# laclouis5/StructureDetector

Hardware: AMD Instinct MI355X
Metric: images/sec (train fwd+bwd) and decode us/img at 512x512 (higher is better)
Workload: dtype f32

## Files before the change

structuredetector_amd/csrc/sd_conv.hip:

```cpp
#include <string.h>
#include "sd_common.h"
#include "sd_mfma.h"
#include "sd_conv_rows.h"

#ifndef SD_S2_LPT
#define SD_S2_LPT 1
#endif
namespace sd {


#ifndef SD_IGEMM_DMA
#define SD_IGEMM_DMA 1
#endif
#ifndef SD_ABLATE_HOT
#define SD_ABLATE_HOT 0
#endif
#ifndef SD_ABLATE_STORE
#define SD_ABLATE_STORE 0
#endif
#ifndef SD_ABLATE_PATCH
#define SD_ABLATE_PATCH 0
#endif
#if SD_ABLATE_HOT || SD_ABLATE_STORE || SD_ABLATE_PATCH || defined(SD_PP_ABL) || defined(SD_RS_ABL)
#warning "timing-only ablation build: this libsdnet_hip.so computes WRONG RESULTS; the Python loader refuses it unless SDNET_ALLOW_ABLATION=1"
#endif
#ifdef SD_DECODE_TRACE
#define SD_TRACE_FLAG 8
#else
#define SD_TRACE_FLAG 0
#endif
#if defined(SD_PP_TRACE) || defined(SD_SB_TRACE)
#undef SD_TRACE_FLAG
#define SD_TRACE_FLAG 8
#endif
#if defined(SD_PP_ABL) || defined(SD_RS_ABL) || defined(SD_SB_ABL) || defined(SD_SHAPE_EXP) || defined(SD_W16_ABL) || defined(SD_SR_ABL) || defined(SD_SF_ABL)
#define SD_EXPERIMENT_FLAG 16
#else
#define SD_EXPERIMENT_FLAG 0
#endif
void sd_nn_set_pool_pair(int v);
extern "C" int sd_build_flags(void) { return (SD_ABLATE_HOT ? 1 : 0) | (SD_ABLATE_STORE ? 2 : 0) | (SD_ABLATE_PATCH ? 4 : 0) | SD_TRACE_FLAG | SD_EXPERIMENT_FLAG; }

#ifndef SD_SHAPE_EXP
#define SD_SHAPE_EXP 0
#else
#define SD_SHAPE_EXP_BUILD 1
#endif
__device__ __forceinline__ f32x16 mfma_shape_exp(bf16x8 a, bf16x8 b, f32x16 c) {
    f32x4 c0 = __builtin_shufflevector(c, c, 0, 1, 2, 3), c1 = __builtin_shufflevector(c, c, 4, 5, 6, 7);
    c0 = __builtin_amdgcn_mfma_f32_16x16x32_bf16(a, b, c0, 0, 0, 0);
    c1 = __builtin_amdgcn_mfma_f32_16x16x32_bf16(b, a, c1, 0, 0, 0);
    c[0] = c0[0]; c[1] = c0[1]; c[2] = c0[2]; c[3] = c0[3]; c[4] = c1[0]; c[5] = c1[1]; c[6] = c1[2]; c[7] = c1[3];
    return c;
}
#define SD_MFMA_BF16(BIT, a, b, c) (((SD_SHAPE_EXP) & (BIT)) ? mfma_shape_exp(a, b, c) : __builtin_amdgcn_mfma_f32_32x32x16_bf16(a, b, c, 0, 0, 0))

#ifndef SD_IGEMM_LATE_DMA
#define SD_IGEMM_LATE_DMA 0
#endif
constexpr int NBUF = 2;
constexpr int BM = 128, BK = 32, LDK = BK;

struct ConvArgs {
    const void* x;
    const void* w;
    void* y;
    const float* scale;
    const float* shift;
    const void* res;
    int B, Hi, Wi, Ck, Ho, Wo, Nn, R, S;
    int mul, div, off, rsign;
    int relu, res_up2;
    int M, nk, kchunks;
    int splits;
    float* part;
    const float* bn_x;
    const float* bn_y;
    const float *bn_mean, *bn_invstd, *bn_gamma, *bn_beta;
    int bn_relu;
    float* stat;
    int pt_tw_log2, pt_pw, pt_pieces, pt_rolling, pt_flip;
    int pt_strip_log2;
    int par;
    const uint16_t* head_w;
    const float* head_b;
    float* head_y;
    int head_co;
};

__device__ __attribute__((aligned(128))) float g_zero_line[64];


__device__ __forceinline__ void s2_tile(int bid, int nwg, int n_tiles, int off, int& cls, int& tq, int& n_idx, int& tile_m) {
    if (SD_S2_LPT && (nwg & 31) == 0) {
        const int xcd = bid & 7, pos = bid >> 3, per = nwg >> 5;
        const int k4 = pos / per, within = xcd * per + (pos - k4 * per);
        cls = (off & 1) ? (k4 == 0 ? 3 : k4 == 3 ? 0 : k4) : k4;
        tq = within / n_tiles; n_idx = within - tq * n_tiles;
    } else {
        const int tile = xcd_remap(bid, nwg), tm = tile / n_tiles;
        cls = tm & 3; tq = tm >> 2; n_idx = tile - tm * n_tiles;
    }
    tile_m = 4 * tq + cls;
}


__device__ __forceinline__ float f4c(const float4& v, int t) { return t == 0 ? v.x : (t == 1 ? v.y : (t == 2 ? v.z : v.w)); }

struct BnRed4 { float4 mu, is, ga, be, s, q; };
__device__ __forceinline__ void bnred4_init(BnRed4& b, const ConvArgs& p, int n) {
    b.mu = *reinterpret_cast<const float4*>(p.bn_mean + n); b.is = *reinterpret_cast<const float4*>(p.bn_invstd + n);
    b.ga = b.be = b.s = b.q = make_float4(0.f, 0.f, 0.f, 0.f);
    if (p.bn_relu == 2) { b.ga = *reinterpret_cast<const float4*>(p.bn_gamma + n); b.be = *reinterpret_cast<const float4*>(p.bn_beta + n); }
}
__device__ __forceinline__ void bnred4_add(BnRed4& b, const ConvArgs& p, float4 g, int64_t m, int n) {
    const int64_t i = m * p.Nn + n;
    const float4 xv = *reinterpret_cast<const float4*>(p.bn_x + i);
    const float4 xh = make_float4((xv.x - b.mu.x) * b.is.x, (xv.y - b.mu.y) * b.is.y, (xv.z - b.mu.z) * b.is.z, (xv.w - b.mu.w) * b.is.w);
    if (p.bn_relu == 1) {
        const float4 yy = *reinterpret_cast<const float4*>(p.bn_y + i);
        g.x = yy.x > 0.f ? g.x : 0.f; g.y = yy.y > 0.f ? g.y : 0.f; g.z = yy.z > 0.f ? g.z : 0.f; g.w = yy.w > 0.f ? g.w : 0.f;
    } else if (p.bn_relu == 3) {
        const uint8_t mb = reinterpret_cast<const uint8_t*>(p.bn_y)[i >> 2];
        g.x = (mb & 1) ? g.x : 0.f; g.y = (mb & 2) ? g.y : 0.f; g.z = (mb & 4) ? g.z : 0.f; g.w = (mb & 8) ? g.w : 0.f;
    } else if (p.bn_relu == 2) {
        g.x = (xh.x * b.ga.x + b.be.x) > 0.f ? g.x : 0.f; g.y = (xh.y * b.ga.y + b.be.y) > 0.f ? g.y : 0.f;
        g.z = (xh.z * b.ga.z + b.be.z) > 0.f ? g.z : 0.f; g.w = (xh.w * b.ga.w + b.be.w) > 0.f ? g.w : 0.f;
    }
    b.s.x += g.x; b.s.y += g.y; b.s.z += g.z; b.s.w += g.w;
    b.q.x += g.x * xh.x; b.q.y += g.y * xh.y; b.q.z += g.z * xh.z; b.q.w += g.w * xh.w;
}
template <int LPR>
__device__ __forceinline__ void bnred4_wave_sum(BnRed4& b) {
#pragma unroll
    for (int o = LPR; o < 64; o <<= 1) {
        b.s.x += __shfl_xor(b.s.x, o); b.s.y += __shfl_xor(b.s.y, o); b.s.z += __shfl_xor(b.s.z, o); b.s.w += __shfl_xor(b.s.w, o);
        b.q.x += __shfl_xor(b.q.x, o); b.q.y += __shfl_xor(b.q.y, o); b.q.z += __shfl_xor(b.q.z, o); b.q.w += __shfl_xor(b.q.w, o);
    }
}

#define SD_BNRED_TERM(v, m, n, S, Q)                                                               \
    {                                                                                              \
        const float xv_ = p.bn_x[(int64_t)(m) * p.Nn + (n)];                                       \
        const float xh_ = (xv_ - bmu) * bis;                                                       \
        float g_ = (v);                                                                            \
        if (p.bn_relu == 1) g_ = p.bn_y[(int64_t)(m) * p.Nn + (n)] > 0.f ? g_ : 0.f;               \
        else if (p.bn_relu == 3) g_ = ((reinterpret_cast<const uint8_t*>(p.bn_y)[((int64_t)(m) * p.Nn + (n)) >> 2] >> ((n) & 3)) & 1) ? g_ : 0.f; \
        else if (p.bn_relu == 2) g_ = (xh_ * bga + bbe) > 0.f ? g_ : 0.f;                          \
        S += g_; Q += g_ * xh_;                                                                    \
    }

template <int BN, int MODE, bool BF16 = false>
__global__ __launch_bounds__(256, 2) void k_conv_igemm(ConvArgs p) {
    constexpr bool STEM = (MODE == 1);
    using T = typename std::conditional<BF16, uint16_t, float>::type;
    constexpr int KE = BF16 ? 64 : 32;
    constexpr int VE = BF16 ? 8 : 4;
    const T* const px_ = reinterpret_cast<const T*>(p.x);
    const T* const pw_ = reinterpret_cast<const T*>(p.w);
    const T* const zero_ = reinterpret_cast<const T*>(g_zero_line);
    constexpr int NT = BN / 64;
    __shared__ __attribute__((aligned(16))) float As0[BM * LDK];
    __shared__ __attribute__((aligned(16))) float As1[BM * LDK];
    __shared__ __attribute__((aligned(16))) float Bs0[BN * LDK];
    __shared__ __attribute__((aligned(16))) float Bs1[BN * LDK];
    __shared__ int orow[BM];
    __shared__ int rrow[BM];

    const int tid = threadIdx.x, lane = tid & 63, wave = tid >> 6;
    const int n_tiles = p.Nn / BN;
    const int tile = xcd_remap(blockIdx.x, gridDim.x);
// ... 4304 lines not shown
    a.pt_rolling = a.Wo == 128;
    a.pt_pw = a.pt_rolling ? 144 : a.Wo + 2;
    a.pt_pieces = a.pt_rolling ? 36 : cdiv((th + 2) * a.pt_pw, 16);
    a.pt_flip = a.rsign < 0;
    return a.pt_pieces * 256 <= (a.pt_rolling ? PT_FLOATS : PT_STAGE_FLOATS);
}

static thread_local int g_patch_narrow = 2;
static int patch_tile_bn(ConvArgs& a, int BN, int mode, bool bf16) {
    ConvArgs t = a;
    if (conv_patch_geometry(t, BN, mode, bf16, false, g_patch_min_tiles)) { a = t; return BN; }
    if (BN == 128 && (bf16 ? g_patch_narrow >= 2 : g_patch_narrow >= 1)) {
        t = a;
        if (conv_patch_geometry(t, 64, mode, bf16, true, g_patch_min_tiles)) { a = t; return 64; }
    }
    return 0;
}

static thread_local int g_rows64_min_units = 192;
static bool conv_rows64_geometry(const ConvArgs& a, int mode, RowsArgs& r) {
    if (mode != 0 || a.Ck != 64 || a.Nn != 64 || a.R != 3 || a.S != 3 || a.mul != 1 || a.div != 1 || a.splits > 1) return false;
    if (!((a.rsign == 1 && a.off == -1) || (a.rsign == -1 && a.off == 1))) return false;
    if (a.Ho != a.Hi || a.Wo != a.Wi || a.Wo % 128 || a.res_up2 || a.bn_x) return false;
    r = RowsArgs{};
    r.B = a.B; r.H = a.Ho; r.W = a.Wo; r.segs = a.Wo / 128;
    const int cols = r.B * r.segs;
    r.rows = std::min(r.H, std::max(8, cdiv(r.H * cols, 256)));
    r.units_per_col = cdiv(r.H, r.rows);
    r.nunits = cols * r.units_per_col;
    if (r.nunits < g_rows64_min_units || (g_rows64_min_units > 1 && r.rows < 16)) return false;
    r.x = (const uint16_t*)a.x; r.w = (const uint16_t*)a.w; r.y = (uint16_t*)a.y; r.scale = a.scale; r.shift = a.shift;
    r.res = (const uint16_t*)a.res; r.stat = a.stat; r.relu = a.relu; r.flip = a.rsign < 0;
    return true;
}

static thread_local int g_rows16 = 1;
static bool conv_rows16_args(const RowsArgs& r) { return g_rows16 && !r.stat; }

static thread_local int g_rowsf32_min_units = 192;
static thread_local int g_stem_fwd_blocks = 512;
static bool conv_rowsf32_geometry(const ConvArgs& a, int mode, RowsArgsF& r) {
    if (mode != 0 || a.Ck != 64 || a.Nn != 64 || a.R != 3 || a.S != 3 || a.mul != 1 || a.div != 1 || a.splits > 1) return false;
    if (!((a.rsign == 1 && a.off == -1) || (a.rsign == -1 && a.off == 1))) return false;
    if (a.Ho != a.Hi || a.Wo != a.Wi || a.Wo % 64 || a.res_up2 || a.bn_x) return false;
    r = RowsArgsF{};
    r.B = a.B; r.H = a.Ho; r.W = a.Wo; r.segs = a.Wo / 64;
    const int cols = r.B * r.segs;
    r.rows = std::min(r.H, std::max(8, cdiv(r.H * cols, 256)));
    r.units_per_col = cdiv(r.H, r.rows);
    r.nunits = cols * r.units_per_col;
    if (r.nunits < g_rowsf32_min_units || (g_rowsf32_min_units > 1 && r.rows < 16)) return false;
    r.x = (const float*)a.x; r.w = (const float*)a.w; r.y = (float*)a.y; r.scale = a.scale; r.shift = a.shift;
    r.res = (const float*)a.res; r.stat = a.stat; r.relu = a.relu; r.flip = a.rsign < 0;
    return true;
}

static thread_local int g_pp_min_tiles = 200;
static thread_local int g_pp_strips = 1;
static bool conv_pp_geometry(ConvArgs& a, int mode, int min_tiles) {
    if (a.Nn % 128 || a.M % PP_BM || (a.M / PP_BM) * (a.Nn / 128) < min_tiles || a.res_up2) return false;
    a.pt_strip_log2 = 0;
    int l2 = 0;
    while ((1 << l2) < a.Wo) ++l2;
    if (g_pp_strips && (1 << l2) == a.Wo && a.Wo >= 128 && a.Wo <= 4096 && a.Ho % 4 == 0) {
        if (!SD_CONV_PATCH || mode != 0 || a.R != 3 || a.S != 3 || a.mul != 1 || a.div != 1 || a.splits > 1) return false;
        if (!((a.rsign == 1 && a.off == -1) || (a.rsign == -1 && a.off == 1))) return false;
        if (a.Ho != a.Hi || a.Wo != a.Wi || a.Ck % 32) return false;
        a.pt_tw_log2 = 6; a.pt_strip_log2 = l2 - 6; a.pt_rolling = 0; a.pt_pw = 66; a.pt_pieces = cdiv(6 * 66, 16); a.pt_flip = a.rsign < 0;
        return true;
    }
    return conv_patch_geometry(a, 128, mode, true, false, 1) && !a.pt_rolling;
}

static thread_local int g_stem_fwd_ring = 1;
static thread_local int g_igemm_big_bf16 = 0;
static int igemm_big_tiles(const ConvArgs& a, int BN, int mode) {
    if (!SD_IGEMM_BIG || (BN != 128 && !SD_IGEMM_BIG64 && !(SD_IGEMM_BIG64_S2 && mode == 2)) || (mode != 0 && mode != 2) || a.splits > 1) return 0;
    if (a.R * a.S * a.Ck < 512) return 0;
    const int m_per = mode == 2 ? a.M / 4 : a.M;
    const int big_tiles = (mode == 2 ? 4 : 1) * cdiv(m_per, BMB) * (a.Nn / BN);
    return (big_tiles >= 512 && (mode != 2 || m_per % BMB == 0)) ? big_tiles : 0;
}

enum ConvFamily {
    CONV_STREAM1X1,
    CONV_ROWS16,
    CONV_ROWS_BF16,
    CONV_ROWS_F32,
    CONV_PP,
    CONV_PP_HEAD,
    CONV_PATCH,
    CONV_PATCH_ROLL,
    CONV_IGEMM_BIG,
    CONV_IGEMM,
};

struct ConvPlan {
    ConvFamily family;
    bool bf16;
    int BN, mode;
    int grid_x, grid_y, block;
    size_t lds;
    int stat_rows;
    ConvArgs a;
    RowsArgs ra;
    RowsArgsF rf;
};

static ConvPlan plan_conv(const ConvArgs& a, bool bf16, bool stem = false) {
    ConvPlan p{};
    p.bf16 = bf16;
    p.a = a;
    p.BN = (a.Nn % 128 == 0) ? 128 : 64;
    p.mode = stem ? 1 : (a.par ? 2 : (a.div > 1 ? 3 : 0));
    p.grid_y = 1; p.block = 256;
    if (!stem && bf16) {
        if (conv1x1_stream_geometry(a, p.mode) && conv1x1_stream_args(a)) {
            p.family = CONV_STREAM1X1;
            p.grid_x = std::min(512, cdiv(a.M / (a.Ck == 64 ? 32 : 16), 4));
            return p;
        }
        if (conv_rows64_geometry(a, p.mode, p.ra)) {
            p.family = conv_rows16_args(p.ra) ? CONV_ROWS16 : CONV_ROWS_BF16;
            p.grid_x = std::min(p.ra.nunits, 256); p.lds = RS_LDS_BYTES; p.stat_rows = p.ra.nunits;
            return p;
        }
        ConvArgs t = a;
        if (conv_pp_geometry(t, p.mode, g_pp_min_tiles)) {
            p.a = t;
            p.family = a.head_y ? CONV_PP_HEAD : CONV_PP;
            p.BN = 128; p.grid_x = (a.M / PP_BM) * (a.Nn / 128); p.block = 512; p.lds = PP_LDS_FLOATS * sizeof(float); p.stat_rows = a.M / PP_BM;
            return p;
        }
    }
    if (!stem && !bf16 && conv_rowsf32_geometry(a, p.mode, p.rf)) {
        p.family = CONV_ROWS_F32;
        p.grid_x = std::min(p.rf.nunits, 256); p.lds = RF_LDS_BYTES; p.stat_rows = p.rf.nunits;
        return p;
    }
    if (!stem) {
        if (const int PBN = patch_tile_bn(p.a, p.BN, p.mode, bf16)) {
            p.family = p.a.pt_rolling ? CONV_PATCH_ROLL : CONV_PATCH;
            p.BN = PBN; p.grid_x = (a.M / BMB) * (a.Nn / PBN); p.stat_rows = cdiv(a.M, BMB);
            return p;
        }
    }
    if (const int big_tiles = (!bf16 || (g_igemm_big_bf16 && p.BN == 128)) ? igemm_big_tiles(a, p.BN, p.mode) : 0) {
        p.family = CONV_IGEMM_BIG;
        p.grid_x = big_tiles; p.stat_rows = cdiv(a.M, BMB);
        return p;
    }
    p.family = CONV_IGEMM;
    p.grid_x = cdiv(a.M, BM) * (a.Nn / p.BN); p.grid_y = a.splits > 1 ? a.splits : 1; p.stat_rows = a.splits > 1 ? 0 : cdiv(a.M, BM);
    return p;
}

static const char* conv_plan_name(const ConvPlan& p, char* buf, size_t n) {
    const char* tf = p.bf16 ? "true" : "false";
    switch (p.family) {
    case CONV_STREAM1X1: return p.a.Ck == 64 ? "k_conv1x1_stream_bf16<64, 2>" : "k_conv1x1_stream_bf16<128, 1>";
    case CONV_ROWS16: return "k_conv3x3_c64_rows16_bf16";
    case CONV_ROWS_BF16: return "k_conv3x3_c64_rows_bf16";
    case CONV_ROWS_F32: return "k_conv3x3_c64_rows_f32";
    case CONV_PP: return "k_conv3x3_bf16_pp";
    case CONV_PP_HEAD: return "k_conv3x3_bf16_pp_head";
    case CONV_PATCH: snprintf(buf, n, "k_conv3x3_patch<%d, %s>", p.BN, tf); return buf;
    case CONV_PATCH_ROLL: snprintf(buf, n, "k_conv3x3_patch_roll<%d, %s>", p.BN, tf); return buf;
    case CONV_IGEMM_BIG: snprintf(buf, n, "k_conv_igemm_big<%d, %d, %s>", p.BN, p.mode, tf); return buf;
    case CONV_IGEMM: snprintf(buf, n, "k_conv_igemm<%d, %d, %s>", p.BN, p.mode, tf); return buf;
    }
    return "";
}

template <auto KERNEL>
static int raise_dynamic_lds(size_t bytes) {
    static thread_local bool raised = false;
    if (!raised) {
        SD_HIP(hipFuncSetAttribute(reinterpret_cast<const void*>(KERNEL), hipFuncAttributeMaxDynamicSharedMemorySize, (int)bytes));
        raised = true;
    }
    return 0;
}

template <int BN, int MODE, bool BF16 = false>
static void launch_tiles(const ConvPlan& p, hipStream_t st) {
    if constexpr ((BN == 128 || (!BF16 && (SD_IGEMM_BIG64 || (SD_IGEMM_BIG64_S2 && MODE == 2)))) && (MODE == 0 || MODE == 2)) {
        if (p.family == CONV_IGEMM_BIG) {
            hipLaunchKernelGGL((k_conv_igemm_big<BN, MODE, BF16>), dim3(p.grid_x), dim3(256), 0, st, p.a);
            return;
        }
    }
    hipLaunchKernelGGL((k_conv_igemm<BN, MODE, BF16>), dim3(p.grid_x, p.grid_y), dim3(256), 0, st, p.a);
}
template <int BN, bool BF16>
static void launch_tiles_mode(const ConvPlan& p, hipStream_t st) {
    if (p.mode == 0) launch_tiles<BN, 0, BF16>(p, st);
    else if (p.mode == 2) launch_tiles<BN, 2, BF16>(p, st);
    else launch_tiles<BN, 3, BF16>(p, st);
}
template <bool BF16>
static void launch_patch(const ConvPlan& p, hipStream_t st) {
    if (p.family == CONV_PATCH_ROLL) {
        if (p.BN == 128) hipLaunchKernelGGL((k_conv3x3_patch_roll<128, BF16>), dim3(p.grid_x), dim3(256), 0, st, p.a);
        else hipLaunchKernelGGL((k_conv3x3_patch_roll<64, BF16>), dim3(p.grid_x), dim3(256), 0, st, p.a);
    } else if (p.BN == 128) hipLaunchKernelGGL((k_conv3x3_patch<128, BF16>), dim3(p.grid_x), dim3(256), 0, st, p.a);
    else hipLaunchKernelGGL((k_conv3x3_patch<64, BF16>), dim3(p.grid_x), dim3(256), 0, st, p.a);
}

static int launch_plan(const ConvPlan& p, hipStream_t st) {
    const ConvArgs& a = p.a;
    SD_REQUIRE(!a.head_y || p.family == CONV_PP_HEAD, SD_ERR_INVALID,
               "sd_conv2d_fwd_bf16_head: this geometry does not take the two-group kernel (ask sd_conv2d_fwd_bf16_head_supported)");
    const dim3 grid(p.grid_x, p.grid_y), block(p.block);
    switch (p.family) {
    case CONV_STREAM1X1:
        if (a.Ck == 64) hipLaunchKernelGGL((k_conv1x1_stream_bf16<64, 2>), grid, block, 0, st, a, a.M / 32);
        else hipLaunchKernelGGL((k_conv1x1_stream_bf16<128, 1>), grid, block, 0, st, a, a.M / 16);
        break;
    case CONV_ROWS16:
    case CONV_ROWS_BF16:
        if (int e = raise_dynamic_lds<k_conv3x3_c64_rows_bf16>(p.lds)) return e;
        if (p.family == CONV_ROWS16) {
            if (int e = launch_rows16_bf16(p.ra, st)) return e;
        } else hipLaunchKernelGGL(k_conv3x3_c64_rows_bf16, grid, block, p.lds, st, p.ra);
        break;
    case CONV_ROWS_F32:
        if (int e = raise_dynamic_lds<k_conv3x3_c64_rows_f32>(p.lds)) return e;
        hipLaunchKernelGGL(k_conv3x3_c64_rows_f32, grid, block, p.lds, st, p.rf);
        break;
    case CONV_PP:
        if (int e = raise_dynamic_lds<k_conv3x3_bf16_pp>(p.lds)) return e;
        hipLaunchKernelGGL(k_conv3x3_bf16_pp, grid, block, p.lds, st, a);
        break;
    case CONV_PP_HEAD:
        if (int e = raise_dynamic_lds<k_conv3x3_bf16_pp_head>(p.lds)) return e;
        hipLaunchKernelGGL(k_conv3x3_bf16_pp_head, grid, block, p.lds, st, a);
        break;
    case CONV_PATCH:
    case CONV_PATCH_ROLL:
        if (p.bf16) launch_patch<true>(p, st); else launch_patch<false>(p, st);
        break;
    case CONV_IGEMM_BIG:
    case CONV_IGEMM:
        if (p.bf16) {
            if (p.BN == 128) launch_tiles_mode<128, true>(p, st); else launch_tiles_mode<64, true>(p, st);
        } else if (p.mode == 1) launch_tiles<64, 1>(p, st);
        else if (p.BN == 128) launch_tiles_mode<128, false>(p, st);
        else launch_tiles_mode<64, false>(p, st);
        break;
    }
    SD_LAUNCH_CHECK();
    if (p.family == CONV_IGEMM && a.splits > 1) {
        if (p.bf16) hipLaunchKernelGGL(k_splitk_reduce<true>, dim3(cdiv((int64_t)a.M * a.Nn / 4, 256)), dim3(256), 0, st, a);
        else hipLaunchKernelGGL(k_splitk_reduce<false>, dim3(cdiv((int64_t)a.M * a.Nn / 4, 256)), dim3(256), 0, st, a);
        SD_LAUNCH_CHECK();
    }
    return 0;
}

static int launch_igemm(const ConvArgs& a, bool stem, hipStream_t st, bool bf16 = false) { return launch_plan(plan_conv(a, bf16, stem), st); }

static thread_local int g_fwd_split_k = 1;
static int fwd_splits(const sd_conv_desc* d, int ke) {
    if (!g_fwd_split_k) return 1;
    const int M = d->B * d->Ho * d->Wo;
    const int BN = (d->Cout % 128 == 0) ? 128 : 64;
    const int tiles = cdiv(M, BM) * (d->Cout / BN);
    const int nk = d->R * d->S * (d->Cin / ke);
    if (tiles >= 256 || nk < 8) return 1;
    int s = std::min(cdiv(512, tiles), nk / 4);
    return std::max(1, std::min(s, 64));
}

static ConvArgs conv_args(const sd_conv_desc* d, int pass, bool bf16) {
    ConvArgs a{};
    const int ke = bf16 ? 64 : BK;
    a.B = d->B; a.R = d->R; a.S = d->S;
    if (pass == 0) {
        a.Hi = d->Hi; a.Wi = d->Wi; a.Ck = d->Cin; a.Ho = d->Ho; a.Wo = d->Wo; a.Nn = d->Cout;
        a.mul = d->stride; a.div = 1; a.off = -d->pad; a.rsign = 1;
        a.splits = fwd_splits(d, ke);
    } else {
        a.Hi = d->Ho; a.Wi = d->Wo; a.Ck = d->Cout; a.Ho = d->Hi; a.Wo = d->Wi; a.Nn = d->Cin;
        a.mul = 1; a.div = d->stride; a.off = d->pad; a.rsign = -1;
    }
    a.M = a.B * a.Ho * a.Wo; a.kchunks = a.Ck / ke; a.nk = a.R * a.S * a.kchunks;
    if (pass == 1) a.par = (d->stride == 2 && d->Hi % 2 == 0 && d->Wi % 2 == 0 && (a.M / 4) % BM == 0) ? 1 : 0;
    return a;
}

static float g_query_operand;
static ConvPlan plan_query(const sd_conv_desc* d, int pass, bool bf16, bool stats) {
    ConvArgs a = conv_args(d, pass, bf16);
    if (stats) { a.stat = &g_query_operand; if (pass == 1) a.bn_x = &g_query_operand; }
    return plan_conv(a, bf16);
}

static int check_conv(const char* what, const sd_conv_desc* d) {
    SD_REQUIRE(d != nullptr, SD_ERR_INVALID, "%s: null descriptor", what);
    SD_REQUIRE(d->B > 0 && d->Hi > 0 && d->Wi > 0 && d->Cin > 0 && d->Cout > 0 && d->R > 0 && d->S > 0 && d->stride > 0 && d->pad >= 0,
// ... 720 lines not shown
    SD_REQUIRE(stem_is_7x7s2(d), SD_ERR_INVALID, "sd_conv2d_stem_wgrad_bf16: the stem is 7x7 / stride 2 / pad 3, 3 -> 64");
    SD_REQUIRE(aligned16(dy_bf16) && aligned16(x_nchw) && d->Wi % 4 == 0, SD_ERR_INVALID,
               "sd_conv2d_stem_wgrad_bf16: dy and the image must be 16-byte aligned and the image width a multiple of 4 (LDS-DMA in 16-byte groups)");
    SD_REQUIRE(workspace_bytes >= sd_conv2d_stem_wgrad_workspace_bytes(d), SD_ERR_WORKSPACE, "sd_conv2d_stem_wgrad_bf16: workspace too small");
    StemArgs a{};
    a.x = x_nchw; a.dy16 = (const uint16_t*)dy_bf16; a.y = (float*)workspace;
    stem_args(a, d);
    a.rg = 64;
    while (a.rg > 8 && d->B * a.tiles_x * cdiv(d->Ho, a.rg) < 512) a.rg >>= 1;
    const int units = d->B * a.tiles_x * cdiv(d->Ho, a.rg);
    const int blocks = std::max(1, std::min(std::min(256, stem_blocks(d)), units));
    hipStream_t st = (hipStream_t)stream;
    static const hipError_t attr_once = hipFuncSetAttribute(reinterpret_cast<const void*>(&k_stem_wgrad_bf16_ring), hipFuncAttributeMaxDynamicSharedMemorySize, (int)SR_LDS_BYTES);
    (void)attr_once;
    hipLaunchKernelGGL(k_stem_wgrad_bf16_ring, dim3(blocks), dim3(256), SR_LDS_BYTES, st, a);
    SD_LAUNCH_CHECK();
    const int64_t n4 = 64 * STEM_K / 4;
    hipLaunchKernelGGL(k_wgrad_reduce_par, dim3(cdiv(n4, 32)), dim3(256), 0, st, (const float*)workspace, dw, n4, blocks, accumulate);
    SD_LAUNCH_CHECK();
    return 0;
}

size_t sd_conv2d_dgrad_bn_reduce_workspace_bytes(const sd_conv_desc* d) {
    if (!d || d->Cin % 64 || d->Cout % 32) return 0;
    const int rows = plan_query(d, 1, false, true).stat_rows;
    return (size_t)(rows + sd_bn_finalize_scratch_rows(rows)) * 2 * d->Cin * sizeof(float);
}

static int conv_dgrad_bn_reduce_any(const char* what, const float* dy, const float* w_t, float* dx, const sd_conv_desc* d, const float* residual,
                                    const float* bn_x, const float* bn_y, int relu, const float* mean, const float* invstd, const float* gamma,
                                    const float* beta, float* dgamma, float* dbeta, int accumulate, float* means_out, double* sums, void* workspace,
                                    size_t workspace_bytes, sd_stream_t stream) {
    if (int e = check_conv(what, d)) return e;
    SD_REQUIRE(dy && w_t && dx && bn_x && mean && invstd && gamma && dgamma && dbeta && (means_out || sums) && workspace, SD_ERR_INVALID,
               "%s: null pointer", what);
    SD_REQUIRE(relu >= 0 && relu <= 3 && ((relu != 1 && relu != 3) || bn_y) && (relu != 2 || beta), SD_ERR_INVALID,
               "%s: relu must be 0, 1 / 3 (need bn_y) or 2 (needs beta)", what);
    SD_REQUIRE(d->Cout % 32 == 0 && d->Cin % 64 == 0, SD_ERR_INVALID, "%s: needs Cout %% 32 == 0 and Cin %% 64 == 0", what);
    SD_REQUIRE(aligned16(dy) && aligned16(w_t) && aligned16(dx) && aligned16(residual) && aligned16(bn_x) && aligned16(bn_y) && aligned16(mean) &&
               aligned16(invstd) && aligned16(gamma) && aligned16(beta) && aligned8(sums), SD_ERR_ALIGN, "%s: pointers must be 16-byte aligned", what);
    SD_REQUIRE(workspace_bytes >= sd_conv2d_dgrad_bn_reduce_workspace_bytes(d), SD_ERR_WORKSPACE, "%s: workspace too small", what);
    ConvArgs a = conv_args(d, 1, false);
    a.x = dy; a.w = w_t; a.y = dx; a.res = residual;
    a.bn_x = bn_x; a.bn_y = bn_y; a.bn_relu = relu; a.bn_mean = mean; a.bn_invstd = invstd; a.bn_gamma = gamma; a.bn_beta = beta;
    a.stat = (float*)workspace;
    const ConvPlan p = plan_conv(a, false);
    if (int e = launch_plan(p, (hipStream_t)stream)) return e;
    const int rows = p.stat_rows;
    if (sums) return sd_bn_bwd_sums((const float*)workspace, rows, (int64_t)a.M, d->Cin, dgamma, dbeta, accumulate, sums,
                                    (float*)workspace + (size_t)rows * 2 * d->Cin, stream);
    return sd_bn_bwd_finalize((const float*)workspace, rows, (int64_t)a.M, d->Cin, dgamma, dbeta, accumulate, means_out,
                              (float*)workspace + (size_t)rows * 2 * d->Cin, stream);
}

int sd_conv2d_dgrad_bn_reduce(const float* dy, const float* w_t, float* dx, const sd_conv_desc* d, const float* residual, const float* bn_x,
                              const float* bn_y, int relu, const float* mean, const float* invstd, const float* gamma, const float* beta,
                              float* dgamma, float* dbeta, int accumulate, float* means_out, void* workspace, size_t workspace_bytes,
                              sd_stream_t stream) {
    SD_REQUIRE(means_out, SD_ERR_INVALID, "sd_conv2d_dgrad_bn_reduce: null pointer");
    return conv_dgrad_bn_reduce_any("sd_conv2d_dgrad_bn_reduce", dy, w_t, dx, d, residual, bn_x, bn_y, relu, mean, invstd, gamma, beta, dgamma, dbeta,
                                    accumulate, means_out, nullptr, workspace, workspace_bytes, stream);
}

int sd_conv2d_dgrad_bn_reduce_sums(const float* dy, const float* w_t, float* dx, const sd_conv_desc* d, const float* residual, const float* bn_x,
                                   const float* bn_y, int relu, const float* mean, const float* invstd, const float* gamma, const float* beta,
                                   float* dgamma, float* dbeta, int accumulate, double* sums, void* workspace, size_t workspace_bytes,
                                   sd_stream_t stream) {
    SD_REQUIRE(sums, SD_ERR_INVALID, "sd_conv2d_dgrad_bn_reduce_sums: null pointer");
    return conv_dgrad_bn_reduce_any("sd_conv2d_dgrad_bn_reduce_sums", dy, w_t, dx, d, residual, bn_x, bn_y, relu, mean, invstd, gamma, beta, dgamma,
                                    dbeta, accumulate, nullptr, sums, workspace, workspace_bytes, stream);
}

#ifdef SD_PP_TRACE
int sd_debug_pp_trace(unsigned long long* out32) { return (int)hipMemcpyFromSymbol(out32, HIP_SYMBOL(sd::g_pp_trace), sizeof(unsigned long long) * 64); }
int sd_debug_stem_trace(unsigned long long* out64) { return (int)hipMemcpyFromSymbol(out64, HIP_SYMBOL(sd::g_stem_trace), sizeof(unsigned long long) * 64); }
int sd_debug_pp_timeline(unsigned long long* out, int blocks) { return (int)hipMemcpyFromSymbol(out, HIP_SYMBOL(sd::g_pp_tl), sizeof(unsigned long long) * 4 * (blocks < 4096 ? blocks : 4096)); }
#endif

int sd_set_option(const char* name, int value) {
    if (name && !strcmp(name, "conv_patch_min_tiles")) { g_patch_min_tiles = value; return 0; }
    if (name && !strcmp(name, "conv_patch_bn64")) { g_patch_bn64 = value; return 0; }
    if (name && !strcmp(name, "conv_pp_min_tiles")) { g_pp_min_tiles = value; return 0; }
    if (name && !strcmp(name, "conv1x1_stream_min_pixels")) { g_conv1x1_stream_min_px = value; return 0; }
    if (name && !strcmp(name, "igemm_big_bf16")) { g_igemm_big_bf16 = value; return 0; }
    if (name && !strcmp(name, "stem_fwd_ring")) { g_stem_fwd_ring = value; return 0; }
    if (name && !strcmp(name, "pool_fwd_pair")) { sd_nn_set_pool_pair(value); return 0; }
    if (name && !strcmp(name, "wgrad_bf16_ring")) { g_wgrad_bf16_ring = value; return 0; }
    if (name && !strcmp(name, "wgrad_f32_ring")) { g_wgrad_f32_ring = value; return 0; }
    if (name && !strcmp(name, "conv_pp_strips")) { g_pp_strips = value; return 0; }
    if (name && !strcmp(name, "conv_patch_narrow")) { g_patch_narrow = value; return 0; }
    if (name && !strcmp(name, "conv_fwd_split_k")) { g_fwd_split_k = value; return 0; }
    if (name && !strcmp(name, "conv_rows64_min_units")) { g_rows64_min_units = value; return 0; }
    if (name && !strcmp(name, "conv_rows16")) { g_rows16 = value; return 0; }
    if (name && !strcmp(name, "conv_rows_f32_min_units")) { g_rowsf32_min_units = value; return 0; }
    if (name && !strcmp(name, "stem_fwd_blocks")) { g_stem_fwd_blocks = value; return 0; }
    sd::set_error("sd_set_option: unknown option '%s'", name ? name : "(null)");
    return SD_ERR_INVALID;
}

const char* sd_conv2d_kernel_name(const sd_conv_desc* d, int pass) {
    static thread_local char name[64];
    if (!d || d->Cin <= 0 || d->Cout <= 0) return "";
    if (pass == 2) {
        const WgradPlan p = plan_wgrad(d, false);
        switch (p.family) {
        case WGRAD_TAPS_RING2: return "k_wgrad3x3_ring2";
        case WGRAD_TAPS_RING: return "k_wgrad3x3_ring";
        case WGRAD_TAPS: return p.roww == 32 ? "k_wgrad3x3<32>" : "k_wgrad3x3<16>";
        default: snprintf(name, sizeof(name), "k_conv_wgrad<%d, %d>", p.TN, p.TC); return name;
        }
    }
    return conv_plan_name(plan_query(d, pass & 15, (pass & 16) != 0, false), name, sizeof(name));
}

}
```

Measured before the change: 872.0.

## Add persistent streaming f32 MFMA kernel for large 1x1 convolutions

Adds a new persistent kernel for f32 1x1 convolutions (stride 1 or 2) and routes large non-bf16 cases to it ahead of the rows/patch/igemm paths. It uses a 4-stage LDS DMA ring with swizzled layout, f32 MFMA, residual prefetch two chunks before the epilogue, and a fused epilogue for BN statistics, scale/shift, residual and relu. The goal is to overlap global loads with compute and amortise launch and tile setup across tiles, in place of the generic implicit-GEMM path. It adds inline-asm wait-count bookkeeping, which risks subtle hazards, and moves ConvArgs into a shared header.

Measured after the change: 874.6, median of 6. No clear change (+0.3%).

```diff
diff --git a/structuredetector_amd/csrc/sd_conv.hip b/structuredetector_amd/csrc/sd_conv.hip
--- a/structuredetector_amd/csrc/sd_conv.hip
+++ b/structuredetector_amd/csrc/sd_conv.hip
@@ -2,6 +2,7 @@
 #include "sd_common.h"
 #include "sd_mfma.h"
 #include "sd_conv_rows.h"
+#include "sd_conv_args.h"
 
 #ifndef SD_S2_LPT
 #define SD_S2_LPT 1
@@ -61,32 +62,6 @@
 constexpr int NBUF = 2;
 constexpr int BM = 128, BK = 32, LDK = BK;
 
-struct ConvArgs {
-    const void* x;
-    const void* w;
-    void* y;
-    const float* scale;
-    const float* shift;
-    const void* res;
-    int B, Hi, Wi, Ck, Ho, Wo, Nn, R, S;
-    int mul, div, off, rsign;
-    int relu, res_up2;
-    int M, nk, kchunks;
-    int splits;
-    float* part;
-    const float* bn_x;
-    const float* bn_y;
-    const float *bn_mean, *bn_invstd, *bn_gamma, *bn_beta;
-    int bn_relu;
-    float* stat;
-    int pt_tw_log2, pt_pw, pt_pieces, pt_rolling, pt_flip;
-    int pt_strip_log2;
-    int par;
-    const uint16_t* head_w;
-    const float* head_b;
-    float* head_y;
-    int head_co;
-};
 
 __device__ __attribute__((aligned(128))) float g_zero_line[64];
 
@@ -4557,8 +4532,20 @@
     return (big_tiles >= 512 && (mode != 2 || m_per % BMB == 0)) ? big_tiles : 0;
 }
 
+static thread_local int g_conv1x1_f32_stream_min_px = 16384;
+static thread_local int g_conv1x1_f32_stream_wide_min_tiles = 256;
+static thread_local int g_conv1x1_f32_stream_blocks = 0;
+static int conv1x1_stream_f32_bn(const ConvArgs& a, int mode) {
+    if (mode != 0 || a.R != 1 || a.S != 1 || a.div != 1 || a.off != 0 || (a.mul != 1 && a.mul != 2) || a.head_y) return 0;
+    if (a.Ck % 64 || a.Nn % 64 || (a.Ck == 512 && a.Nn == 512) || a.M < g_conv1x1_f32_stream_min_px) return 0;
+    if (a.bn_x || a.res_up2 > 1 || (a.res_up2 == 1 && (a.Ho % 2 || a.Wo % 2))) return 0;
+    if (a.stat && (a.splits > 1 || igemm_big_tiles(a, a.Nn % 128 == 0 ? 128 : 64, mode))) return 0;
+    return (a.Nn % 128 == 0 && cdiv(a.M, 128) * (a.Nn / 128) >= g_conv1x1_f32_stream_wide_min_tiles) ? 128 : 64;
+}
+
 enum ConvFamily {
     CONV_STREAM1X1,
+    CONV_STREAM1X1_F32,
     CONV_ROWS16,
     CONV_ROWS_BF16,
     CONV_ROWS_F32,
@@ -4608,6 +4595,13 @@
             return p;
         }
     }
+    if (!stem && !bf16) {
+        if (const int SBN = conv1x1_stream_f32_bn(a, p.mode)) {
+            p.family = CONV_STREAM1X1_F32;
+            p.BN = SBN; p.a.splits = 1; p.grid_x = 0; p.stat_rows = cdiv(a.M, BM);
+            return p;
+        }
+    }
     if (!stem && !bf16 && conv_rowsf32_geometry(a, p.mode, p.rf)) {
         p.family = CONV_ROWS_F32;
         p.grid_x = std::min(p.rf.nunits, 256); p.lds = RF_LDS_BYTES; p.stat_rows = p.rf.nunits;
@@ -4634,6 +4628,7 @@
     const char* tf = p.bf16 ? "true" : "false";
     switch (p.family) {
     case CONV_STREAM1X1: return p.a.Ck == 64 ? "k_conv1x1_stream_bf16<64, 2>" : "k_conv1x1_stream_bf16<128, 1>";
+    case CONV_STREAM1X1_F32: return p.BN == 128 ? "k_conv1x1_stream_f32<128>" : "k_conv1x1_stream_f32<64>";
     case CONV_ROWS16: return "k_conv3x3_c64_rows16_bf16";
     case CONV_ROWS_BF16: return "k_conv3x3_c64_rows_bf16";
     case CONV_ROWS_F32: return "k_conv3x3_c64_rows_f32";
@@ -4691,6 +4686,9 @@
     case CONV_STREAM1X1:
         if (a.Ck == 64) hipLaunchKernelGGL((k_conv1x1_stream_bf16<64, 2>), grid, block, 0, st, a, a.M / 32);
         else hipLaunchKernelGGL((k_conv1x1_stream_bf16<128, 1>), grid, block, 0, st, a, a.M / 16);
+        break;
+    case CONV_STREAM1X1_F32:
+        if (int e = launch_conv1x1_stream_f32(a, p.BN, g_conv1x1_f32_stream_blocks, st)) return e;
         break;
     case CONV_ROWS16:
     case CONV_ROWS_BF16:
@@ -5577,6 +5575,9 @@
     if (name && !strcmp(name, "conv_patch_bn64")) { g_patch_bn64 = value; return 0; }
     if (name && !strcmp(name, "conv_pp_min_tiles")) { g_pp_min_tiles = value; return 0; }
     if (name && !strcmp(name, "conv1x1_stream_min_pixels")) { g_conv1x1_stream_min_px = value; return 0; }
+    if (name && !strcmp(name, "conv1x1_f32_stream_min_pixels")) { g_conv1x1_f32_stream_min_px = value; return 0; }
+    if (name && !strcmp(name, "conv1x1_f32_stream_wide_min_tiles")) { g_conv1x1_f32_stream_wide_min_tiles = value; return 0; }
+    if (name && !strcmp(name, "conv1x1_f32_stream_blocks")) { g_conv1x1_f32_stream_blocks = value; return 0; }
     if (name && !strcmp(name, "igemm_big_bf16")) { g_igemm_big_bf16 = value; return 0; }
     if (name && !strcmp(name, "stem_fwd_ring")) { g_stem_fwd_ring = value; return 0; }
     if (name && !strcmp(name, "pool_fwd_pair")) { sd_nn_set_pool_pair(value); return 0; }
diff --git a/structuredetector_amd/csrc/sd_conv1x1_f32.hip b/structuredetector_amd/csrc/sd_conv1x1_f32.hip
--- /dev/null
+++ b/structuredetector_amd/csrc/sd_conv1x1_f32.hip
@@ -0,0 +1,319 @@
+#include <algorithm>
+#include "sd_common.h"
+#include "sd_mfma.h"
+#include "sd_conv_args.h"
+
+namespace sd {
+
+constexpr int S1_BM = 128, S1_BK = 16, S1_NST = 4, S1_PAW = 2;
+
+static __device__ __attribute__((aligned(128))) float g_s1_zero_line[64];
+
+constexpr int s1_vmcnt_imm(int n) { return (n & 15) | (7 << 4) | (15 << 8) | ((n >> 4) << 14); }
+
+__device__ __forceinline__ f32x4 s1_load16_async(const float* src) {
+    f32x4 v = {0.f, 0.f, 0.f, 0.f};
+#if defined(__HIP_DEVICE_COMPILE__)
+    asm volatile("global_load_dwordx4 %0, %1, off" : "=&v"(v) : "v"(src) : "memory");
+#else
+    (void)src;
+#endif
+    return v;
+}
+template <int N>
+__device__ __forceinline__ void s1_wait_loads(f32x4 (&r)[16]) {
+#if defined(__HIP_DEVICE_COMPILE__)
+    asm volatile("s_waitcnt %16"
+                 : "+v"(r[0]), "+v"(r[1]), "+v"(r[2]), "+v"(r[3]), "+v"(r[4]), "+v"(r[5]), "+v"(r[6]), "+v"(r[7]), "+v"(r[8]), "+v"(r[9]),
+                   "+v"(r[10]), "+v"(r[11]), "+v"(r[12]), "+v"(r[13]), "+v"(r[14]), "+v"(r[15])
+                 : "n"(s1_vmcnt_imm(N))
+                 : "memory");
+#endif
+}
+template <int N>
+__device__ __forceinline__ void s1_wait_loads(f32x4 (&r)[8]) {
+#if defined(__HIP_DEVICE_COMPILE__)
+    asm volatile("s_waitcnt %8"
+                 : "+v"(r[0]), "+v"(r[1]), "+v"(r[2]), "+v"(r[3]), "+v"(r[4]), "+v"(r[5]), "+v"(r[6]), "+v"(r[7])
+                 : "n"(s1_vmcnt_imm(N))
+                 : "memory");
+#endif
+}
+__device__ __forceinline__ void s1_lds_barrier() {
+#if defined(__HIP_DEVICE_COMPILE__)
+    asm volatile("s_waitcnt lgkmcnt(0)\n\ts_barrier" ::: "memory");
+#endif
+}
+
+template <int OFF>
+__device__ __forceinline__ void s1_lds_write32(uint32_t addr, float v) {
+#if defined(__HIP_DEVICE_COMPILE__)
+    asm volatile("ds_write_b32 %0, %1 offset:%2" :: "v"(addr), "v"(v), "n"(OFF) : "memory");
+#else
+    (void)addr; (void)v;
+#endif
+}
+__device__ __forceinline__ float s1_lds_read32(uint32_t addr) {
+    float v = 0.f;
+#if defined(__HIP_DEVICE_COMPILE__)
+    asm volatile("ds_read_b32 %0, %1\n\ts_waitcnt lgkmcnt(0)" : "=v"(v) : "v"(addr) : "memory");
+#else
+    (void)addr;
+#endif
+    return v;
+}
+
+template <int BN, bool FULL, int NS>
+__device__ __forceinline__ void s1_epilogue(const ConvArgs& p, f32x16 (&acc)[2][BN / 64], f32x4 (&R)[NS], uint32_t T, uint32_t statred,
+                                            int m0, int n0, int tile_m, const f32x4 sc4, const f32x4 sh4, int wave, int lane) {
+    constexpr int WC = BN / 2, NTW = WC / 32, LPR = WC / 4, RPI = 64 / LPR, IPP = 8 / RPI;
+    const int fr = lane & 31, fh = lane >> 5;
+    const int wm0 = (wave >> 1) * 64, wn0 = (wave & 1) * WC;
+    if (p.stat) {
+        float sv[NTW], qv[NTW];
+#pragma unroll
+        for (int ni = 0; ni < NTW; ++ni) {
+            sv[ni] = qv[ni] = 0.f;
+#pragma unroll
+            for (int mi = 0; mi < 2; ++mi)
+#pragma unroll
+                for (int e = 0; e < 16; ++e) { const float a = acc[mi][ni][e]; sv[ni] += a; qv[ni] += a * a; }
+            sv[ni] += __shfl_xor(sv[ni], 32); qv[ni] += __shfl_xor(qv[ni], 32);
+            if ((wave >> 1) == 1 && fh == 0) { s1_lds_write32<0>(statred + (wn0 + ni * 32 + fr) * 4, sv[ni]); s1_lds_write32<BN * 4>(statred + (wn0 + ni * 32 + fr) * 4, qv[ni]); }
+        }
+        s1_lds_barrier();
+        if ((wave >> 1) == 0 && fh == 0) {
+            float* dst = p.stat + (int64_t)tile_m * 2 * p.Nn + n0;
+#pragma unroll
+            for (int ni = 0; ni < NTW; ++ni) {
+                const int c = wn0 + ni * 32 + fr;
+                dst[c] = sv[ni] + s1_lds_read32(statred + c * 4); dst[p.Nn + c] = qv[ni] + s1_lds_read32(statred + (BN + c) * 4);
+            }
+        }
+    }
+    const int c4 = (lane % LPR) * 4;
+    float* const yb = reinterpret_cast<float*>(p.y) + n0 + wn0 + c4;
+    const uint32_t tw = T + ((4 * fh) * WC + fr) * 4, tr = T + ((lane / LPR) * WC + c4) * 4;
+#pragma unroll
+    for (int mi = 0; mi < 2; ++mi)
+#pragma unroll
+        for (int b = 0; b < 4; ++b) {
+#pragma unroll
+            for (int ni = 0; ni < NTW; ++ni)
+            {
+                const f32x16& c = acc[mi][ni];
+                if (ni == 0) {
+                    s1_lds_write32<0>(tw, c[4 * b]); s1_lds_write32<WC * 4>(tw, c[4 * b + 1]);
+                    s1_lds_write32<2 * WC * 4>(tw, c[4 * b + 2]); s1_lds_write32<3 * WC * 4>(tw, c[4 * b + 3]);
+                } else {
+                    s1_lds_write32<32 * 4>(tw, c[4 * b]); s1_lds_write32<(WC + 32) * 4>(tw, c[4 * b + 1]);
+                    s1_lds_write32<(2 * WC + 32) * 4>(tw, c[4 * b + 2]); s1_lds_write32<(3 * WC + 32) * 4>(tw, c[4 * b + 3]);
+                }
+            }
+            f32x4 t0 = lds_read128_async<0>(tr), t1 = t0;
+            if (IPP == 2) t1 = lds_read128_async<RPI * WC * 4>(tr);
+            SD_LDS_WAIT2(0, t0, t1);
+#pragma unroll
+            for (int it = 0; it < IPP; ++it) {
+                const int rl = it * RPI + lane / LPR;
+                const int m = m0 + wm0 + mi * 32 + b * 8 + rl;
+                const f32x4 tv = it == 0 ? t0 : t1;
+                float4 v = make_float4(tv[0], tv[1], tv[2], tv[3]);
+                v.x = v.x * sc4[0] + sh4[0]; v.y = v.y * sc4[1] + sh4[1]; v.z = v.z * sc4[2] + sh4[2]; v.w = v.w * sc4[3] + sh4[3];
+                if (p.res) {
+                    const f32x4 r = R[(mi * 4 + b) * IPP + it];
+                    v.x += r[0]; v.y += r[1]; v.z += r[2]; v.w += r[3];
+                }
+                if (p.relu) { v.x = fmaxf(v.x, 0.f); v.y = fmaxf(v.y, 0.f); v.z = fmaxf(v.z, 0.f); v.w = fmaxf(v.w, 0.f); }
+                if (FULL || m < p.M) *reinterpret_cast<float4*>(yb + (int64_t)m * p.Nn) = v;
+            }
+        }
+}
+
+template <int BN>
+__global__ __launch_bounds__(256, 2) void k_conv1x1_stream_f32(ConvArgs p, int total_tiles) {
+    constexpr int WC = BN / 2, NTW = WC / 32, PBW = BN / 64, PW = S1_PAW + PBW;
+    constexpr int A_ST = S1_BM * S1_BK, ST = A_ST + BN * S1_BK;
+    constexpr int LPR = WC / 4, RPI = 64 / LPR, IPP = 8 / RPI, NS = 8 * IPP;
+    static_assert(BN == 128 || BN == 64, "wave tile 64 x 64 or 64 x 32");
+    __shared__ __attribute__((aligned(16))) float ring[S1_NST * ST];
+    __shared__ __attribute__((aligned(16))) float epi[4][8 * WC];
+    __shared__ __attribute__((aligned(16))) float statred[2][BN];
+    __shared__ int rrow[2][S1_BM];
+    const float* const x = reinterpret_cast<const float*>(p.x);
+    const float* const w = reinterpret_cast<const float*>(p.w);
+    const float* const res = reinterpret_cast<const float*>(p.res);
+
+    const int tid = threadIdx.x, lane = tid & 63, wave = __builtin_amdgcn_readfirstlane(tid >> 6);
+    const int G = gridDim.x, vb = xcd_remap(blockIdx.x, G);
+    const int n_tiles = p.Nn / BN, nkc = p.Ck / S1_BK;
+    const int nmine = (total_tiles - vb + G - 1) / G;
+    const int nchunks = nmine * nkc;
+    const int HWo = p.Ho * p.Wo;
+
+    const int prow = lane >> 2, pslot = lane & 3;
+    const int qe = (pslot ^ ((prow >> 2) & 3)) * 4;
+    const float* const zsrc = g_s1_zero_line + qe;
+    auto src_of = [&](int m) -> const float* {
+        if (m >= p.M) return nullptr;
+        int64_t pix = m;
+        if (p.mul != 1) {
+            const int b = m / HWo, r = m - b * HWo, oy = r / p.Wo, ox = r - oy * p.Wo;
+            pix = ((int64_t)b * p.Hi + oy * p.mul) * p.Wi + ox * p.mul;
+        }
+        return x + pix * p.Ck + qe;
+    };
+    int i_tile = vb, i_kc = 0, i_stage = 0, i_left = nchunks;
+    const float *a0 = nullptr, *a1 = nullptr, *b0 = zsrc, *b1 = zsrc;
+    auto issue = [&]() {
+        float* const dst = ring + i_stage * ST;
+        if (i_left > 0) {
+            if (i_kc == 0) {
+                const int tm = i_tile / n_tiles, ni = i_tile - tm * n_tiles;
+                const int r0 = tm * S1_BM + wave * 32 + prow;
+                a0 = src_of(r0); a1 = src_of(r0 + 16);
+                b0 = w + (int64_t)(ni * BN + wave * (PBW * 16) + prow) * p.Ck + qe; b1 = b0 + 16 * p.Ck;
+            }
+            const int ko = i_kc * S1_BK;
+            lds_dma16(a0 ? a0 + ko : zsrc, dst + (wave * 2) * 256);
+            lds_dma16(a1 ? a1 + ko : zsrc, dst + (wave * 2 + 1) * 256);
+            lds_dma16(b0 + ko, dst + A_ST + (wave * PBW) * 256);
+            if (PBW == 2) lds_dma16(b1 + ko, dst + A_ST + (wave * PBW + 1) * 256);
+            if (++i_kc == nkc) { i_kc = 0; i_tile += G; }
+            --i_left;
+        } else {
+#pragma unroll
+            for (int j = 0; j < PW; ++j) lds_dma16(zsrc, dst + (j < 2 ? (wave * 2 + j) * 256 : A_ST + (wave * PBW + j - 2) * 256));
+        }
+        i_stage = i_stage == S1_NST - 1 ? 0 : i_stage + 1;
+    };
+
+    const int wm0 = (wave >> 1) * 64, wn0 = (wave & 1) * WC;
+    const int fr = lane & 31, fh = lane >> 5;
+    const int rd_swz = (fr >> 2) & 3;
+    const uint32_t ring_base = lds_addr(ring), epi_addr = lds_addr(epi[wave]), statred_addr = lds_addr(statred);
+    const uint32_t a_k0 = ((wm0 + fr) * S1_BK + (((0 + fh) ^ rd_swz) << 2)) * 4, a_k1 = ((wm0 + fr) * S1_BK + (((2 + fh) ^ rd_swz) << 2)) * 4;
+    const uint32_t b_k0 = (A_ST + (wn0 + fr) * S1_BK + (((0 + fh) ^ rd_swz) << 2)) * 4, b_k1 = (A_ST + (wn0 + fr) * S1_BK + (((2 + fh) ^ rd_swz) << 2)) * 4;
+    constexpr int TSTR = 32 * S1_BK * 4;
+
+    f32x16 acc[2][NTW];
+#pragma unroll
+    for (int mi = 0; mi < 2; ++mi)
+#pragma unroll
+        for (int ni = 0; ni < NTW; ++ni)
+#pragma unroll
+            for (int e = 0; e < 16; ++e) acc[mi][ni][e] = 0.f;
+    f32x4 R[NS];
+#pragma unroll
+    for (int s = 0; s < NS; ++s) R[s] = f32x4{0.f, 0.f, 0.f, 0.f};
+
+    const int c4 = (lane % LPR) * 4;
+    int n0 = (vb % n_tiles) * BN;
+    f32x4 sc4 = {1.f, 1.f, 1.f, 1.f}, sh4 = {0.f, 0.f, 0.f, 0.f};
+    if (p.scale) sc4 = s1_load16_async(p.scale + n0 + wn0 + c4);
+    if (p.shift) sh4 = s1_load16_async(p.shift + n0 + wn0 + c4);
+#if defined(__HIP_DEVICE_COMPILE__)
+    asm volatile("s_waitcnt vmcnt(0)" : "+v"(sc4), "+v"(sh4) :: "memory");
+#endif
+
+    issue(); issue(); issue();
+    wait_vmcnt<2 * PW>();
+    __builtin_amdgcn_s_barrier();
+
+    int tile = vb, kc = 0, stage = 0, par = 0;
+    bool counted_stores = false;
+    for (int g = 0; g < nchunks; ++g) {
+        const int tile_m = tile / n_tiles, m0 = tile_m * S1_BM;
+        const bool last = kc == nkc - 1, early = kc == nkc - 2;
+        if (kc == 0 && res && p.res_up2 && tid < S1_BM) {
+            const int m = m0 + tid;
+            int rm = 0;
+            if (m < p.M) {
+                const int b = m / HWo, r = m - b * HWo, oy = r / p.Wo, ox = r - oy * p.Wo;
+                rm = (b * (p.Ho >> 1) + (oy >> 1)) * (p.Wo >> 1) + (ox >> 1);
+            }
+            rrow[par][tid] = rm;
+        }
+        if (early && res) {
+            const float* const rb = res + n0 + wn0 + c4;
+#pragma unroll
+            for (int s = 0; s < NS; ++s) {
+                const int row = wm0 + (s / (4 * IPP)) * 32 + ((s / IPP) & 3) * 8 + (s % IPP) * RPI + lane / LPR;
+                const int m = m0 + row;
+                const int64_t rm = p.res_up2 ? rrow[par][row] : (m < p.M ? m : 0);
+                R[s] = s1_load16_async(rb + rm * p.Nn);
+            }
+        }
+        issue();
+        {
+            const uint32_t sb = ring_base + stage * (ST * 4);
+            f32x4 a00 = lds_read128_async<0>(sb + a_k0), a01 = lds_read128_async<TSTR>(sb + a_k0);
+            f32x4 b00 = lds_read128_async<0>(sb + b_k0), b01 = b00;
+            if (NTW == 2) b01 = lds_read128_async<TSTR>(sb + b_k0);
+            f32x4 a10 = lds_read128_async<0>(sb + a_k1), a11 = lds_read128_async<TSTR>(sb + a_k1);
+            f32x4 b10 = lds_read128_async<0>(sb + b_k1), b11 = b10;
+            if (NTW == 2) b11 = lds_read128_async<TSTR>(sb + b_k1);
+            if (NTW == 2) { SD_LDS_WAIT4(4, a00, a01, b00, b01); } else { asm volatile("s_waitcnt lgkmcnt(3)" : "+v"(a00), "+v"(a01), "+v"(b00) :: "memory"); }
+#pragma unroll
+            for (int t = 0; t < 4; ++t) {
+                acc[0][0] = __builtin_amdgcn_mfma_f32_32x32x2f32(a00[t], b00[t], acc[0][0], 0, 0, 0);
+                acc[1][0] = __builtin_amdgcn_mfma_f32_32x32x2f32(a01[t], b00[t], acc[1][0], 0, 0, 0);
+                if (NTW == 2) {
+                    acc[0][NTW - 1] = __builtin_amdgcn_mfma_f32_32x32x2f32(a00[t], b01[t], acc[0][NTW - 1], 0, 0, 0);
+                    acc[1][NTW - 1] = __builtin_amdgcn_mfma_f32_32x32x2f32(a01[t], b01[t], acc[1][NTW - 1], 0, 0, 0);
+                }
+            }
+            if (NTW == 2) { SD_LDS_WAIT4(0, a10, a11, b10, b11); } else { asm volatile("s_waitcnt lgkmcnt(0)" : "+v"(a10), "+v"(a11), "+v"(b10) :: "memory"); }
+#pragma unroll
+            for (int t = 0; t < 4; ++t) {
+                acc[0][0] = __builtin_amdgcn_mfma_f32_32x32x2f32(a10[t], b10[t], acc[0][0], 0, 0, 0);
+                acc[1][0] = __builtin_amdgcn_mfma_f32_32x32x2f32(a11[t], b10[t], acc[1][0], 0, 0, 0);
+                if (NTW == 2) {
+                    acc[0][NTW - 1] = __builtin_amdgcn_mfma_f32_32x32x2f32(a10[t], b11[t], acc[0][NTW - 1], 0, 0, 0);
+                    acc[1][NTW - 1] = __builtin_amdgcn_mfma_f32_32x32x2f32(a11[t], b11[t], acc[1][NTW - 1], 0, 0, 0);
+                }
+            }
+        }
+        if (((last || early) && res) || (kc < 2 && counted_stores)) wait_vmcnt_and_lds<2 * PW + NS>();
+        else wait_vmcnt_and_lds<2 * PW>();
+        __builtin_amdgcn_s_barrier();
+        stage = stage == S1_NST - 1 ? 0 : stage + 1;
+        if (last) {
+            if (res) s1_wait_loads<2 * PW>(R);
+            const bool full = m0 + S1_BM <= p.M;
+            if (full) s1_epilogue<BN, true, NS>(p, acc, R, epi_addr, statred_addr, m0, n0, tile_m, sc4, sh4, wave, lane);
+            else s1_epilogue<BN, false, NS>(p, acc, R, epi_addr, statred_addr, m0, n0, tile_m, sc4, sh4, wave, lane);
+            counted_stores = full && !p.stat;
+#pragma unroll
+            for (int mi = 0; mi < 2; ++mi)
+#pragma unroll
+                for (int ni = 0; ni < NTW; ++ni)
+#pragma unroll
+                    for (int e = 0; e < 16; ++e) acc[mi][ni][e] = 0.f;
+            kc = 0; tile += G; par ^= 1;
+            if (n_tiles > 1 && g + 1 < nchunks) {
+                n0 = (tile % n_tiles) * BN;
+                if (p.scale) sc4 = s1_load16_async(p.scale + n0 + wn0 + c4);
+                if (p.shift) sh4 = s1_load16_async(p.shift + n0 + wn0 + c4);
+            }
+        } else ++kc;
+    }
+    wait_vmcnt<0>();
+}
+
+int launch_conv1x1_stream_f32(const ConvArgs& a, int BN, int blocks, hipStream_t st) {
+    static thread_local int cus = 0;
+    if (blocks <= 0 && !cus) {
+        int dev = 0;
+        SD_HIP(hipGetDevice(&dev));
+        SD_HIP(hipDeviceGetAttribute(&cus, hipDeviceAttributeMultiprocessorCount, dev));
+    }
+    const int total = cdiv(a.M, S1_BM) * (a.Nn / BN);
+    const int grid = std::min(total, blocks > 0 ? blocks : 2 * cus);
+    if (BN == 128) hipLaunchKernelGGL(k_conv1x1_stream_f32<128>, dim3(grid), dim3(256), 0, st, a, total);
+    else hipLaunchKernelGGL(k_conv1x1_stream_f32<64>, dim3(grid), dim3(256), 0, st, a, total);
+    SD_LAUNCH_CHECK();
+    return 0;
+}
+
+}
diff --git a/structuredetector_amd/csrc/sd_conv_args.h b/structuredetector_amd/csrc/sd_conv_args.h
--- /dev/null
+++ b/structuredetector_amd/csrc/sd_conv_args.h
@@ -0,0 +1,36 @@
+#pragma once
+#include <stdint.h>
+#include <hip/hip_runtime.h>
+
+namespace sd {
+
+struct ConvArgs {
+    const void* x;
+    const void* w;
+    void* y;
+    const float* scale;
+    const float* shift;
+    const void* res;
+    int B, Hi, Wi, Ck, Ho, Wo, Nn, R, S;
+    int mul, div, off, rsign;
+    int relu, res_up2;
+    int M, nk, kchunks;
+    int splits;
+    float* part;
+    const float* bn_x;
+    const float* bn_y;
+    const float *bn_mean, *bn_invstd, *bn_gamma, *bn_beta;
+    int bn_relu;
+    float* stat;
+    int pt_tw_log2, pt_pw, pt_pieces, pt_rolling, pt_flip;
+    int pt_strip_log2;
+    int par;
+    const uint16_t* head_w;
+    const float* head_b;
+    float* head_y;
+    int head_co;
+};
+
+int launch_conv1x1_stream_f32(const ConvArgs& a, int BN, int blocks, hipStream_t st);
+
+}
```
